# Wu0409/DuPL

Measured on AMD Instinct MI355X. Metric: training img/s at 448^2, VOC dual-student ViT-B/16, phase B step, higher is better.
Workload: dtype f32 storage / accumulation / results; Linear GEMMs (forward, dgrad, wgrad), attention (forward, backward) and the decoder convs as fp32-equivalent f16x3 split products on the f16 MFMA (operands as fp16 hi / lo planes, 3 products per block, fp32 accumulate; error vs fp64 <= the f32 MFMA kernels'); CA

## Files before the change

### dupl_amd/csrc/gemm_split.hip

```cpp
#include "common.h"
#include <type_traits>
#include "../../include/dupl_hip.h"

#ifndef G16_ABL
#define G16_ABL 0
#endif

namespace {

typedef _Float16 h8 __attribute__((ext_vector_type(8)));

constexpr int TBK = 32;
constexpr float LO_INV = 1.f / DUPL_LO_SCALE;

template <bool F1>
__global__ __launch_bounds__(256) void split_kernel(const float* __restrict__ x, __half* __restrict__ hi, __half* __restrict__ lo,
                                                    long n4, float scale) {
    for (long i = (long)blockIdx.x * blockDim.x + threadIdx.x; i < n4; i += (long)gridDim.x * blockDim.x) {
        const float4 v = reinterpret_cast<const float4*>(x)[i];
        __half h[4], l[4];
        if constexpr (F1) {
            split_f32_u(v.x * scale, h[0], l[0]);
            split_f32_u(v.y * scale, h[1], l[1]);
            split_f32_u(v.z * scale, h[2], l[2]);
// ... 44 lines not shown
#pragma unroll
            for (int e = 0; e < 16; ++e) {
                int row = rbase + (e & 3) + 8 * (e >> 2);
                asm volatile("" : "+v"(row));
                if (!interior && row >= p.M) continue;
                float v = (accM[i][j][e] + accX[i][j][e] * LO_INV) * alpha + bv;
                const bool w32 = p.c_rows <= 0 || row < p.c_rows;
                if (f_pre && w32) p.aux[(size_t)row * p.ldaux + col] = v;
                if (f_gelu) v = gelu_f(v);
                if (f_relu) v = fmaxf(v, 0.f);
                if (f_dgelu) v *= gelu_grad_f(p.aux[(size_t)row * p.ldaux + col]);
                if (f_rmask) v = p.aux[(size_t)row * p.ldaux + col] > 0.f ? v : 0.f;
                if (p.res) v += p.res[(size_t)row * p.ldr + col];
                if (f_acc) {
                    float* cp = p.C + (size_t)row * p.ldc + col;
                    if (ksplit > 1) unsafeAtomicAdd(cp, v);
                    else *cp += v;
                    continue;
                }
                amx = fmaxf(amx, fabsf(v));
                if (p.C && w32) p.C[(size_t)row * p.ldc + col] = v;
                if (Ch) {
                    __half h, l;
                    split_f32(v, h, l);
                    Ch[(size_t)row * p.ldo + col] = h;
                    Cl[(size_t)row * p.ldo + col] = l;
                }
            }
        }
    }
}


template <int WM, int WN, int WMP, bool SINGLE>
__device__ __forceinline__ void gemm16_epilogue_lds(const dupl_gemm16_desc& p, f32x16 (&accM)[WM][WN], f32x16 (&accX)[SINGLE ? 1 : WM][SINGLE ? 1 : WN],
                                                    float* __restrict__ tile, const int mw0, const int nw, const int lane,
                                                    const int ksplit, float& amx) {
    constexpr int TW = 32 * WN, TH = 32 * WMP, LPR = TW / 4, RPI = 64 / LPR;
    static_assert(WM % WMP == 0, "passes");
    const int l31 = lane & 31, hf = lane >> 5;
    const int fl = p.flags;
    const bool f_pre = fl & DUPL_GEMM_STORE_PRE, f_gelu = fl & DUPL_GEMM_GELU, f_relu = fl & DUPL_GEMM_RELU;
    const bool f_acc = fl & DUPL_GEMM_ACCUM, f_dgelu = fl & DUPL_GEMM_MUL_DGELU, f_rmask = fl & DUPL_GEMM_MUL_RELUMASK;
    const float alpha = (p.alpha_dev ? *p.alpha_dev : 1.f) * (p.post_scale != 0.f ? p.post_scale : 1.f);
    const float out_scale = p.out_exp > 0 ? ldexpf(1.f, p.out_exp) : 0.f;
#pragma unroll
    for (int ps = 0; ps < WM / WMP; ++ps) {
    const int mw = mw0 + ps * TH;
#pragma unroll
    for (int i = 0; i < WMP; ++i)
#pragma unroll
        for (int j = 0; j < WN; ++j)
#pragma unroll
            for (int e = 0; e < 16; ++e) {
                float v;
                if constexpr (SINGLE) v = accM[ps * WMP + i][j][e] * alpha;
                else v = (accM[ps * WMP + i][j][e] + accX[ps * WMP + i][j][e] * LO_INV) * alpha;
                tile[(i * 32 + (e & 3) + 8 * (e >> 2) + 4 * hf) * TW + j * 32 + l31] = v;
            }
    __half* Ch = static_cast<__half*>(p.C_hi);
    __half* Cl = static_cast<__half*>(p.C_lo);
    auto a16 = [](const void* q) { return (reinterpret_cast<uintptr_t>(q) & 15) == 0; };
    const bool vec = !(p.N & 3) && !(p.ldc & 3) && !(p.ldo & 3) && !(p.ldr & 3) && !(p.ldaux & 3) && a16(p.C) && a16(p.res) &&
                     a16(p.aux) && a16(p.bias) && !(reinterpret_cast<uintptr_t>(Ch) & 7) && !(reinterpret_cast<uintptr_t>(Cl) & 7);
    if (f_acc) {
        constexpr int RPA = 64 / TW;
        const int ca = lane % TW, ra = lane / TW;
        if (nw + ca >= p.N) continue;
        for (int r = ra; r < TH; r += RPA) {
            const int row = mw + r;
            if (row >= p.M) break;
            float* cp = p.C + (size_t)row * p.ldc + nw + ca;
            const float v = tile[r * TW + ca];
            if (ksplit > 1) unsafeAtomicAdd(cp, v);
            else *cp += v;
        }
        continue;
    }
    const int cl = (lane % LPR) * 4, rl = lane / LPR;
    const int col = nw + cl;
    const int nv = min(4, p.N - col);
    if (nv <= 0) continue;
    float bv[4] = {0.f, 0.f, 0.f, 0.f};
    if (p.bias) {
#pragma unroll
        for (int c = 0; c < 4; ++c)
            if (c < nv) bv[c] = p.bias[col + c];
    }
    const bool fast = vec && nv == 4;
    constexpr int EPU = 4;
    const bool need_aux = f_dgelu | f_rmask;
    for (int r0 = rl; r0 < TH; r0 += EPU * RPI) {
        f32x4 rq[EPU], aq[EPU];
        if (fast) {
#pragma unroll
            for (int u = 0; u < EPU; ++u) {
                const int r = r0 + u * RPI, row = mw + r;
                if (r < TH && row < p.M) {
                    if (p.res) rq[u] = *reinterpret_cast<const f32x4*>(p.res + (size_t)row * p.ldr + col);
                    if (need_aux) aq[u] = *reinterpret_cast<const f32x4*>(p.aux + (size_t)row * p.ldaux + col);
                }
            }
        }
#pragma unroll
        for (int u = 0; u < EPU; ++u) {
        const int r = r0 + u * RPI;
        if (r >= TH) break;
        const int row = mw + r;
        if (row >= p.M) break;
        const f32x4 t = *reinterpret_cast<const f32x4*>(tile + r * TW + cl);
        if (G16_ABL & 4) {
            if (t[0] + t[1] + t[2] + t[3] == 123.456f) p.C[0] = 1.f;
            continue;
        }
        float v[4] = {t[0] + bv[0], t[1] + bv[1], t[2] + bv[2], t[3] + bv[3]};
        float* auxp = p.aux + (size_t)row * p.ldaux + col;
        const bool w32 = p.c_rows <= 0 || row < p.c_rows;
        if (f_pre && w32) {
            if (fast) *reinterpret_cast<f32x4*>(auxp) = f32x4{v[0], v[1], v[2], v[3]};
            else
                {
_Pragma("unroll") for (int c = 0; c < 4; ++c) if (c < nv) auxp[c] = v[c]; }
        }
        if (f_gelu) gelu4(v);
        if (f_relu) {
#pragma unroll
            for (int c = 0; c < 4; ++c) v[c] = fmaxf(v[c], 0.f);
        }
        if (need_aux) {
            float a[4] = {0.f, 0.f, 0.f, 0.f};
            if (fast) {
                a[0] = aq[u][0]; a[1] = aq[u][1]; a[2] = aq[u][2]; a[3] = aq[u][3];
            } else
                {
_Pragma("unroll") for (int c = 0; c < 4; ++c) if (c < nv) a[c] = auxp[c]; }
            if (f_dgelu) gelu_grad_mul4(v, a);
            else {
#pragma unroll
                for (int c = 0; c < 4; ++c) v[c] = a[c] > 0.f ? v[c] : 0.f;
            }
        }
        if (p.res) {
            const float* rp = p.res + (size_t)row * p.ldr + col;
// ... 9 lines not shown
        if (p.C && w32) {
            float* cp = p.C + (size_t)row * p.ldc + col;
            if (fast) *reinterpret_cast<f32x4*>(cp) = f32x4{v[0], v[1], v[2], v[3]};
            else
                {
_Pragma("unroll") for (int c = 0; c < 4; ++c) if (c < nv) cp[c] = v[c]; }
        }
        if (Ch) {
            __half h[4], l[4];
            if (out_scale > 0.f) {
#pragma unroll
                for (int c = 0; c < 4; ++c) split_f32_u(v[c] * out_scale, h[c], l[c]);
            } else {
#pragma unroll
                for (int c = 0; c < 4; ++c) split_f32(v[c], h[c], l[c]);
            }
            __half* hp = Ch + (size_t)row * p.ldo + col;
            __half* lp = Cl + (size_t)row * p.ldo + col;
            if (fast) {
                *reinterpret_cast<uint2*>(hp) = *reinterpret_cast<const uint2*>(h);
                *reinterpret_cast<uint2*>(lp) = *reinterpret_cast<const uint2*>(l);
            } else
                {
_Pragma("unroll") for (int c = 0; c < 4; ++c)
                    if (c < nv) {
                        hp[c] = h[c];
                        lp[c] = l[c];
                    }
                }
        }
        }
    }
    }
}


struct Epi16 {
    bool f_pre, f_gelu, f_relu, f_dgelu, f_rmask, vec;
    float out_scale;
    __half *Ch, *Cl;
};
__device__ __forceinline__ Epi16 epi16_setup(const dupl_gemm16_desc& p) {
    Epi16 e;
    const int fl = p.flags;
    e.f_pre = fl & DUPL_GEMM_STORE_PRE; e.f_gelu = fl & DUPL_GEMM_GELU; e.f_relu = fl & DUPL_GEMM_RELU;
    e.f_dgelu = fl & DUPL_GEMM_MUL_DGELU; e.f_rmask = fl & DUPL_GEMM_MUL_RELUMASK;
    e.Ch = static_cast<__half*>(p.C_hi);
    e.Cl = static_cast<__half*>(p.C_lo);
    e.out_scale = p.out_exp > 0 ? ldexpf(1.f, p.out_exp) : 0.f;
    auto a16 = [](const void* q) { return (reinterpret_cast<uintptr_t>(q) & 15) == 0; };
    e.vec = !(p.N & 3) && !(p.ldc & 3) && !(p.ldo & 3) && !(p.ldr & 3) && !(p.ldaux & 3) && a16(p.C) && a16(p.res) && a16(p.aux) &&
            a16(p.bias) && !(reinterpret_cast<uintptr_t>(e.Ch) & 7) && !(reinterpret_cast<uintptr_t>(e.Cl) & 7);
    return e;
}
__device__ __forceinline__ void epi16_quad(const dupl_gemm16_desc& p, const Epi16& E, const int row, const int col, const int nv,
                                           const f32x4 t, const float (&bv)[4], float& amx, const f32x4 pre = f32x4{0.f, 0.f, 0.f, 0.f},
                                           const int pre_kind = 0) {
    const bool fast = E.vec && nv == 4;
    float v[4] = {t[0] + bv[0], t[1] + bv[1], t[2] + bv[2], t[3] + bv[3]};
    float* auxp = p.aux + (size_t)row * p.ldaux + col;
    const bool w32 = p.c_rows <= 0 || row < p.c_rows;
    if (E.f_pre && w32) {
        if (fast) *reinterpret_cast<f32x4*>(auxp) = f32x4{v[0], v[1], v[2], v[3]};
        else {
#pragma unroll
            for (int c = 0; c < 4; ++c) if (c < nv) auxp[c] = v[c];
// ... 217 lines not shown
            const int cs = s == 0 ? c0 : c1;
            h8 ah[WM], al[WM], bh[WN], bl[WN];
#pragma unroll
            for (int i = 0; i < WM; ++i) {
                ah[i] = *reinterpret_cast<const h8*>(st + a_row + i * 2048 + cs);
                al[i] = *reinterpret_cast<const h8*>(st + PA * 1024 + a_row + i * 2048 + cs);
            }
#pragma unroll
            for (int j = 0; j < WN; ++j) {
                bh[j] = *reinterpret_cast<const h8*>(st + b_row + j * 2048 + cs);
                bl[j] = *reinterpret_cast<const h8*>(st + PB * 1024 + b_row + j * 2048 + cs);
            }
#pragma unroll
            for (int i = 0; i < WM; ++i)
#pragma unroll
                for (int j = 0; j < WN; ++j) {
                    accM[i][j] = __builtin_amdgcn_mfma_f32_32x32x16_f16(ah[i], bh[j], accM[i][j], 0, 0, 0);
                    accX[i][j] = __builtin_amdgcn_mfma_f32_32x32x16_f16(ah[i], bl[j], accX[i][j], 0, 0, 0);
                    accX[i][j] = __builtin_amdgcn_mfma_f32_32x32x16_f16(al[i], bh[j], accX[i][j], 0, 0, 0);
                }
        }
    }

    float amx = 0.f;
    gemm16_epilogue<WM, WN>(p, accM, accX, m0 + wm * (32 * WM), n0 + wn * (32 * WN), m0 + BM <= p.M && n0 + BN <= p.N, l31, hf,
                            ksplit, amx);
    if (p.amax_out)
        gemm16_amax_flush(static_cast<unsigned int*>(p.amax_out), amx, reinterpret_cast<float*>(smem), threadIdx.x >> 6,
                          threadIdx.x & 63, NWM * NWN);
}


#define WAIT_LGKM0_VM(n) ((((n) & 15) | (((n) >> 4) << 14)) | (7 << 4))

template <int NMF, int NR, int R = 0>
__device__ __forceinline__ void sched_mfma_ds() {
    if constexpr (R < NR) {
        constexpr int nm = (R + 1) * NMF / NR - R * NMF / NR;
        if constexpr (nm > 0) __builtin_amdgcn_sched_group_barrier(0x008, nm, 0);
        __builtin_amdgcn_sched_group_barrier(0x100, 1, 0);
        sched_mfma_ds<NMF, NR, R + 1>();
    }
}
template <int NMF, int NR, int ND, int S = 0, int RD = 0, int DD = 0>
__device__ __forceinline__ void sched_mfma_ds_dma() {
    constexpr int NS = NR + ND;
    if constexpr (S < NS) {
        constexpr int nm = (S + 1) * NMF / NS - S * NMF / NS;
        if constexpr (nm > 0) __builtin_amdgcn_sched_group_barrier(0x008, nm, 0);
        constexpr bool rd = RD < NR && (DD >= ND || RD * ND <= DD * NR);
        if constexpr (rd) {
            __builtin_amdgcn_sched_group_barrier(0x100, 1, 0);
            sched_mfma_ds_dma<NMF, NR, ND, S + 1, RD + 1, DD>();
        } else {
            __builtin_amdgcn_sched_group_barrier(0x010, 1, 0);
            sched_mfma_ds_dma<NMF, NR, ND, S + 1, RD, DD + 1>();
        }
    }
}

template <int NR, int ND, int RD = 0, int DD = 0, class FR, class FD, class A, class B>
__device__ __forceinline__ void loads_b(FR& read_item, FD& dma_item, const char* st, const int cs, A& fa, B& fb, char* dst) {
    if constexpr (RD + DD < NR + ND) {
        constexpr bool rd = RD < NR && (DD >= ND || RD * ND <= DD * NR);
        if constexpr (rd) {
            read_item(std::integral_constant<int, RD>{}, st, cs, fa, fb);
// ... 187 lines not shown
        rb = nb;
    }

    asm volatile("s_waitcnt lgkmcnt(0)" ::: "memory");
    __builtin_amdgcn_s_barrier();
    asm volatile("" ::: "memory");
    constexpr int WMP = (NW * (32 * WM) * (32 * WN) * 4 <= STAGES * STAGE) ? WM : WM / 2;
    static_assert(NW * (32 * WMP) * (32 * WN) * 4 <= STAGES * STAGE, "epilogue tiles must fit the stages");
    if (G16_ABL & 16)
        if (tid == 0 && p.aux) reinterpret_cast<long long*>(p.aux)[(size_t)(blockIdx.x + gridDim.x * blockIdx.y) * 8 + 2] = clock64();
    if (G16_ABL & 8) {
        float sum = 0.f;
#pragma unroll
        for (int i = 0; i < WM; ++i)
#pragma unroll
            for (int j = 0; j < WN; ++j)
#pragma unroll
                for (int e = 0; e < 16; ++e) sum += accM[i][j][e] + (SINGLE ? 0.f : accX[SINGLE ? 0 : i][SINGLE ? 0 : j][e]);
        if (sum == 123.456f) p.C[0] = 1.f;
        return;
    }
    float amx = 0.f;
    gemm16_epilogue_lds<WM, WN, WMP, SINGLE>(p, accM, accX, reinterpret_cast<float*>(smem) + wave * ((32 * WMP) * (32 * WN)),
                                             m0 + wm * (32 * WM), n0 + wn * (32 * WN), lane, ksplit, amx);
    if (p.amax_out) gemm16_amax_flush(static_cast<unsigned int*>(p.amax_out), amx, reinterpret_cast<float*>(smem), wave, lane, NWM * NWN);
    if (G16_ABL & 16) {
        asm volatile("s_waitcnt vmcnt(0)" ::: "memory");
        if (tid == 0 && p.aux) {
            long long* q = reinterpret_cast<long long*>(p.aux) + (size_t)(blockIdx.x + gridDim.x * blockIdx.y) * 8;
            q[3] = clock64();
            q[5] = wall_clock64();
        }
    }
}


template <int WM, int WN, int NWM, int NWN, int WPS, bool SK = false, bool SINGLE = false, int STAGES = 3>
__global__ __launch_bounds__(64 * NWM * NWN, WPS) void gemm_f16x3_pring_kernel(const dupl_gemm16_desc p, const int g_gm) {
    constexpr int BM = 32 * WM * NWM, BN = 32 * WN * NWN, NW = NWM * NWN;
    constexpr int PA = BM / 16, PB = BN / 16;
    constexpr int NP = 2 * PA + 2 * PB;
    constexpr int STAGE = NP * 1024;
    constexpr int PPW = NP / NW;
    constexpr int NMF = 3 * WM * WN, NR = 2 * (WM + WN);
    constexpr int SIDE = NW * 2048;
    static_assert(NP % NW == 0, "pieces must divide over the waves");
    static_assert(STAGES * STAGE + SIDE <= 160 * 1024, "LDS");
    __shared__ __attribute__((aligned(1024))) char smem[STAGES * STAGE + SIDE];
    const int tid = threadIdx.x;
    const int lane = tid & 63, wave = __builtin_amdgcn_readfirstlane(tid >> 6);
    const int wm = wave / NWN, wn = wave % NWN;
    const int l31 = lane & 31, hf = lane >> 5;
    const int nbm = (p.M + BM - 1) / BM, nbn = (p.N + BN - 1) / BN;
    const int nblk = nbm * nbn;
    const int ntf = p.K / TBK;
    int nt = ntf;
    const int q8 = nblk >> 3, r8 = nblk & 7;
    const int gspan = g_gm * nbn;
    auto lid_origin = [&](const int lid, int& m0, int& n0) __attribute__((always_inline)) {
        const int gid = lid / gspan, gin = lid - gid * gspan;
        const int gfirst = gid * g_gm;
        const int gsz = min(nbm - gfirst, g_gm);
        m0 = (gfirst + gin % gsz) * BM;
        n0 = (gin / gsz) * BN;
    };
    auto tile_origin = [&](const int bid, int& m0, int& n0) __attribute__((always_inline)) {
// ... 164 lines not shown
        const int mw = m0 + wm * (32 * WM), nw = n0 + wn * (32 * WN);
        bool more;
        if constexpr (SK) {
            pos += nt;
            more = pos < pend;
            if (more) {
                nt = min(pend - pos, ntf);
                lid_origin(pos / ntf, m0, n0);
                plan(m0, n0, 0);
            }
        } else {
            bid += gridDim.x;
            more = has_tile(bid);
            if (more) {
                tile_origin(bid, m0, n0);
                plan(m0, n0, 0);
            }
        }
        if (more) {
#pragma unroll
            for (int s = 0; s < STAGES; ++s) issue(s);
        }
        gemm16_epilogue_side<WM, WN, SK, SINGLE>(p, accM, accX, reinterpret_cast<float*>(smem + STAGES * STAGE) + wave * 512, mw, nw, lane,
                                         amx);
        if (!more) break;
    }
    if (p.amax_out)
        gemm16_amax_flush(static_cast<unsigned int*>(p.amax_out), amx, reinterpret_cast<float*>(smem + STAGES * STAGE), wave, lane,
                          NWM * NWN);
}

typedef short s4v __attribute__((ext_vector_type(4)));
typedef _Float16 h4 __attribute__((ext_vector_type(4)));
template <int N, int I = 0, class F>
__device__ __forceinline__ void static_for(F&& f) {
    if constexpr (I < N) {
        f(std::integral_constant<int, I>{});
        static_for<N, I + 1>(f);
    }
}

constexpr bool slot_is_read(int S, int NR, int ND) {
    int rd = 0, dd = 0;
    for (int s = 0;; ++s) {
        const bool r = rd < NR && (dd >= ND || rd * ND <= dd * NR);
        if (s == S) return r;
        if (r) ++rd; else ++dd;
    }
}
constexpr int slot_index(int S, int NR, int ND) {
    int rd = 0, dd = 0;
    for (int s = 0;; ++s) {
        const bool r = rd < NR && (dd >= ND || rd * ND <= dd * NR);
        if (s == S) return r ? rd : dd;
        if (r) ++rd; else ++dd;
    }
}

template <int WM, int WN, int NWM, int NWN, int WPS, bool SK, int ACC, bool AKM, bool BKM, int STAGES = 3, bool ONESHOT = false>
__device__ __forceinline__ void gemm_f16x3_km_body(const dupl_gemm16_desc& p, const int g_gm, const int bid0, const int grid) {
    constexpr int BM = 32 * WM * NWM, BN = 32 * WN * NWN, NW = NWM * NWN;
    constexpr int PA = BM / 16, PB = BN / 16;
    constexpr int NP = 2 * PA + 2 * PB;
    constexpr int STAGE = NP * 1024;
    constexpr int PPW = NP / NW;
    constexpr int APW = 2 * PA / NW;
    constexpr int RBA = 2 * BM, RBB = 2 * BN;
    constexpr int NDA = AKM ? 2 : 1, NDB = BKM ? 2 : 1;
    constexpr int NIA = 2 * WM * NDA, NIB = 2 * WN * NDB;
    constexpr int NRI = NIA + NIB;
    constexpr int NMF = 3 * WM * WN;
    constexpr int SIDE = NW * 2048;
    static_assert(NP % NW == 0 && (2 * PA) % NW == 0, "pieces must divide over the waves, operand by operand");
    static_assert(STAGES * STAGE + SIDE <= 160 * 1024, "LDS");
// ... 346 lines not shown
                       ldexpf(1.f, scale_exp));
    return dupl_launch_status();
}

extern "C" int dupl_gemm_f16x3_group(const dupl_gemm16_desc* descs, int32_t n, dupl_stream_t stream) {
    if (!descs || n < 1 || n > DUPL_GEMM16_GROUP_MAX) return DUPL_ERR_ARG;
    g16_group_args g;
    g.n = n;
    int total = 0, group = 0;
    auto al16 = [](const void* q) { return (reinterpret_cast<uintptr_t>(q) & 15) == 0; };
    for (int i = 0; i < n; ++i) {
        const dupl_gemm16_desc& d = descs[i];
        if (d.struct_size != sizeof(dupl_gemm16_desc)) return DUPL_ERR_ARG;
        if (!d.A_hi || !d.A_lo || !d.B_hi || !d.B_lo || !d.C || d.C_hi || d.C_lo || d.bias || d.res || d.c_rows || d.amax_out ||
            d.M <= 0 || d.N <= 0 || d.K <= 0)
            return DUPL_ERR_ARG;
        if (d.flags != DUPL_GEMM_ACCUM || d.fmt != 1 || d.a_layout != 1 || d.b_layout != 1 || (d.K % TBK) || d.K / TBK < 3 ||
            (d.lda % 8) || (d.ldb % 8) || (d.M & 7) || (d.N & 7) || d.ka_valid < 0 || d.kb_valid < 0 || d.ka_valid > d.K ||
            d.kb_valid > d.K || d.group < 0 || d.group > 4096)
            return DUPL_ERR_ARG;
        if (!al16(d.A_hi) || !al16(d.A_lo) || !al16(d.B_hi) || !al16(d.B_lo)) return DUPL_ERR_ARG;
        g.d[i] = d;
        g.first[i] = total;
        const int nblk = ((d.M + 255) / 256) * ((d.N + 127) / 128);
        total += nblk;
        if (d.group) group = d.group;
    }
    g.first[n] = total;
    DUPL_LAUNCH((gemm_f16x3_km_group_kernel<2, 2, 4, 2, 2>), dim3((unsigned)(8 * ((total + 7) / 8))), dim3(512), 0, (hipStream_t)stream, g,
                       group ? group : G16_GROUP_RING);
    return dupl_launch_status();
}

extern "C" int dupl_gemm_f16x3(const dupl_gemm16_desc* d, dupl_stream_t stream) {
    if (!d || d->struct_size != sizeof(dupl_gemm16_desc)) return DUPL_ERR_ARG;
    if (!d->A_hi || !d->A_lo || !d->B_hi || !d->B_lo || d->M <= 0 || d->N <= 0 || d->K <= 0) return DUPL_ERR_ARG;
    if ((d->K % TBK) || (d->lda % 8) || (d->ldb % 8)) return DUPL_ERR_ARG;
    if (d->tile < 0 || d->concurrency < 0 || d->concurrency > 8 || d->group < 0 || d->group > 4096 || d->persist_blocks < 0 ||
        d->persist_blocks > 1024 || (d->persist_blocks & 7))
        return DUPL_ERR_ARG;
    {
        const int t = d->tile;
        if (t != 0 && t != 3 && t != 5 && t != 6 && t != 7 && t != 8 && t != 10 && t != 11 && t != 12 && t != 14) return DUPL_ERR_ARG;
    }
    const int g16_tile = d->tile, g16_concurrency = d->concurrency > 0 ? d->concurrency : 1;
    const int g16_persist_blocks = d->persist_blocks ? d->persist_blocks : (g16_concurrency >= 2 ? 192 : 256);
    const int g16_group_m = d->group ? d->group : G16_GROUP_M, g16_group_ring = d->group ? d->group : G16_GROUP_RING;
    const int g16_f1_big_from = G16_F1_BIG_FROM;
    auto al16 = [](const void* q) { return (reinterpret_cast<uintptr_t>(q) & 15) == 0; };
    if (!al16(d->A_hi) || !al16(d->A_lo) || !al16(d->B_hi) || !al16(d->B_lo)) return DUPL_ERR_ARG;
    if (!d->C && !d->C_hi) return DUPL_ERR_ARG;
    if ((d->C_hi == nullptr) != (d->C_lo == nullptr)) return DUPL_ERR_ARG;
    if ((d->flags & (DUPL_GEMM_STORE_PRE | DUPL_GEMM_MUL_DGELU | DUPL_GEMM_MUL_RELUMASK)) && !d->aux) return DUPL_ERR_ARG;
    if (d->flags & ~(DUPL_GEMM_GELU | DUPL_GEMM_RELU | DUPL_GEMM_STORE_PRE | DUPL_GEMM_ACCUM | DUPL_GEMM_MUL_DGELU |
                     DUPL_GEMM_MUL_RELUMASK))
        return DUPL_ERR_ARG;
    const bool accum = d->flags & DUPL_GEMM_ACCUM;
    if (accum && (!d->C || d->C_hi || d->bias || d->res || d->c_rows)) return DUPL_ERR_ARG;
    if (d->c_rows < 0 || (d->c_rows && (d->flags & (DUPL_GEMM_MUL_DGELU | DUPL_GEMM_MUL_RELUMASK)))) return DUPL_ERR_ARG;
    if (d->amax_out && (accum || d->c_rows || (reinterpret_cast<uintptr_t>(d->amax_out) & 3))) return DUPL_ERR_ARG;
    const bool kmajor = d->a_layout || d->b_layout;
    if (d->fmt < 0 || d->fmt > 1 || d->out_exp < 0 || d->out_exp > 15 || (d->out_exp && d->fmt != 1) ||
        (d->fmt == 1 && !kmajor && (accum || d->amax_out)))
        return DUPL_ERR_ARG;
    hipStream_t s = (hipStream_t)stream;
    int ksplit = 1;
    if (accum) {
        const long tiles = (long)((d->M + 127) / 128) * ((d->N + 127) / 128);
        ksplit = (int)((512 + tiles - 1) / tiles);
        const int maxs = (d->K / TBK + 7) / 8;
        if (ksplit > maxs) ksplit = maxs;
        if (ksplit < 1) ksplit = 1;
        if (d->deterministic) ksplit = 1;
    }
    int tile = g16_tile;
    if (tile == 0) {
// ... 19 lines not shown
        if ((d->a_layout ? d->ka_valid : 0) > d->K || (d->b_layout ? d->kb_valid : 0) > d->K) return DUPL_ERR_ARG;
        if (!d->a_layout && d->ka_valid) return DUPL_ERR_ARG;
        if (!d->b_layout && d->kb_valid) return DUPL_ERR_ARG;
        const int nb21 = ((d->M + 255) / 256) * ((d->N + 127) / 128);
        const bool sk = accum && !d->deterministic && ksplit > 1;
        dupl_gemm16_desc dsk = *d;
        if (accum) {
            const int ntf = d->K / TBK;
            auto per = [&](int s_) { return (ntf + s_ - 1) / s_; };
            auto fits = [&](int s_) { return s_ > 0 && (long)nb21 * s_ <= g16_persist_blocks && per(s_) >= 3 && ntf - (s_ - 1) * per(s_) >= 3; };
            if (dsk.sk_slices > 0 && !fits(dsk.sk_slices)) dsk.sk_slices = 0;
            if (dsk.sk_slices == 0) {
                int S = nb21 > g16_persist_blocks ? -1 : g16_persist_blocks / nb21;
                while (S > 1 && (per(S) < 3 || ntf - (S - 1) * per(S) < 3)) --S;
                dsk.sk_slices = S;
            }
            if (dsk.sk_slices > 0 && !fits(dsk.sk_slices)) dsk.sk_slices = -1;
        }
        if (accum && !d->a_layout) {
            if (!d->b_layout || d->deterministic) return DUPL_ERR_ARG;
            DUPL_LAUNCH((gemm_f16x3_km_kernel<2, 2, 4, 2, 2, true, 1, false, true>), dim3((unsigned)g16_persist_blocks), dim3(512), 0, s, dsk, g16_group_ring);
        } else if (accum) {
            if (!(d->a_layout && d->b_layout)) return DUPL_ERR_ARG;
            if (sk) DUPL_LAUNCH((gemm_f16x3_km_kernel<2, 2, 4, 2, 2, true, 1, true, true>), dim3((unsigned)g16_persist_blocks), dim3(512), 0, s, dsk, g16_group_ring);
            else DUPL_LAUNCH((gemm_f16x3_km_kernel<2, 2, 4, 2, 2, false, 2, true, true>), persist_grid(nb21), dim3(512), 0, s, *d, g16_group_ring);
        } else {
            if (d->a_layout || !d->b_layout) return DUPL_ERR_ARG;
            DUPL_LAUNCH((gemm_f16x3_km_kernel<2, 2, 4, 2, 2, false, 0, false, true>), persist_grid(nb21), dim3(512), 0, s, *d, g16_group_ring);
        }
        return dupl_launch_status();
    }
    if (d->fmt == 1) {
        const int nb22 = ((d->M + 255) / 256) * ((d->N + 255) / 256), nb21 = ((d->M + 255) / 256) * ((d->N + 127) / 128);
        int t = (g16_tile == 8 || g16_tile == 12 || g16_tile == 14) ? g16_tile : (nb22 >= g16_f1_big_from ? 8 : 12);
        if (d->K / TBK < 3 && t == 14) t = 12;
        if (t == 8) {
            const int cn = (d->N + 255) / 256, rm = (d->M + 255) / 256, cus = 256;
            const int full = nb22 / cus, tail = nb22 - full * cus;
            const int r_big = full > 0 ? (full * cus) / cn : 0;
            if (g16_tile == 0 && full > 0 && tail > 0 && tail * 10 < cus * 3 && r_big > 0 && r_big < rm && !d->amax_out) {
                const int M1 = r_big * 256;
                dupl_gemm16_desc d1 = *d, d2 = *d;
                d1.M = M1;
                d2.M = d->M - M1;
                auto adv = [&](const void* q, size_t elems, size_t bytes) { return q ? static_cast<const void*>(static_cast<const char*>(q) + elems * bytes) : nullptr; };
                d2.A_hi = adv(d->A_hi, (size_t)M1 * d->lda, 2); d2.A_lo = adv(d->A_lo, (size_t)M1 * d->lda, 2);
                d2.C = (float*)adv(d->C, (size_t)M1 * d->ldc, 4);
                d2.C_hi = (void*)adv(d->C_hi, (size_t)M1 * d->ldo, 2); d2.C_lo = (void*)adv(d->C_lo, (size_t)M1 * d->ldo, 2);
                d2.res = (const float*)adv(d->res, (size_t)M1 * d->ldr, 4);
                d2.aux = (float*)adv(d->aux, (size_t)M1 * d->ldaux, 4);
                if (d->c_rows > 0) {
                    if (d->c_rows <= M1) {
                        d2.c_rows = 0; d2.C = nullptr; d2.aux = nullptr; d2.flags &= ~DUPL_GEMM_STORE_PRE;
                    } else { d1.c_rows = 0; d2.c_rows = d->c_rows - M1; }
                }
                if (d2.C || d2.C_hi) {
                    DUPL_LAUNCH((gemm_f16x3_ring_kernel<4, 2, 2, 4, 2, 2, true>), dim3((unsigned)(r_big * cn)), dim3(512), 0, s, d1, g16_group_ring);
                    DUPL_LAUNCH((gemm_f16x3_ring_kernel<2, 2, 4, 2, 2, 3, true>),
                                       dim3((unsigned)(((d2.M + 255) / 256) * ((d2.N + 127) / 128))), dim3(512), 0, s, d2, g16_group_ring);
                    return dupl_launch_status();
                }
            }
            DUPL_LAUNCH((gemm_f16x3_ring_kernel<4, 2, 2, 4, 2, 2, true>), blocks(256, 256), dim3(512), 0, s, *d, g16_group_ring);
        }
        else if (t == 12) DUPL_LAUNCH((gemm_f16x3_ring_kernel<2, 2, 4, 2, 2, 3, true>), blocks(256, 128), dim3(512), 0, s, *d, g16_group_ring);
        else
            DUPL_LAUNCH((gemm_f16x3_pring_kernel<2, 2, 4, 2, 2, false, true, 3>), persist_grid(nb21), dim3(512), 0, s, *d, g16_group_ring);
        return dupl_launch_status();
    }
    if (tile == 10 && (accum || d->K / TBK < 3)) tile = 6;
    if (tile == 11 && (!accum || d->deterministic || d->K / TBK < 8)) tile = accum ? 5 : 6;
    if (tile == 11) {
        DUPL_LAUNCH((gemm_f16x3_pring_kernel<2, 2, 4, 2, 2, true>), dim3((unsigned)g16_persist_blocks), dim3(512), 0, s, *d,
                           g16_group_ring);
        return dupl_launch_status();
    }
    if (tile == 10) {
        const int nblk = ((d->M + 255) / 256) * ((d->N + 127) / 128);
        const int tx = (nblk + 7) / 8, bmax = g16_persist_blocks / 8;
        const int rounds = (tx + bmax - 1) / bmax;
        const int grid = 8 * ((tx + rounds - 1) / rounds);
        DUPL_LAUNCH((gemm_f16x3_pring_kernel<2, 2, 4, 2, 2>), dim3((unsigned)grid), dim3(512), 0, s, *d, g16_group_ring);
        return dupl_launch_status();
    }
    if (tile == 8 || tile == 9 || tile == 12 || tile == 14) tile = 5;
    if (tile == 6) DUPL_LAUNCH((gemm_f16x3_ring_kernel<2, 2, 4, 2, 2>), blocks(256, 128), dim3(512), 0, s, *d, g16_group_ring);
    else if (tile == 7) DUPL_LAUNCH((gemm_f16x3_ring_kernel<4, 2, 2, 2, 1>), blocks(256, 128), dim3(256), 0, s, *d, g16_group_ring);
    else if (tile == 3) DUPL_LAUNCH((gemm_f16x3_kernel<2, 1, 2, 2, 2>), blocks(128, 64), dim3(256), 0, s, *d, g16_group_m);
    else DUPL_LAUNCH((gemm_f16x3_kernel<2, 1, 2, 4, 4>), blocks(128, 128), dim3(512), 0, s, *d, g16_group_m);
    return dupl_launch_status();
}
```

Baseline: 77.83.

## Add 16x16x32 MFMA ring GEMM kernel for fmt1 split-f16 path and make it default

Adds a new ring-buffered f16x3 GEMM kernel that uses 16x16x32 f16 MFMA instructions. It has its own LDS layout, a phase-interleaved fragment schedule with sched_group_barrier hints, and a rotated LDS epilogue to reduce bank conflicts. It becomes the default for the fmt==1 GEMMs, including the row-split big/tail launch, and the old kernels stay reachable via tiles 8 and 12. The shared epilogue is refactored into a row writer with a pluggable park step. The intent is higher MFMA throughput and better LDS/compute overlap, at the risk of register pressure or a worse schedule than the tuned 32x32 kernel.

New measurement: 80.54, median of 6. 1.03x the previous value.

```diff
diff --git a/dupl_amd/csrc/gemm_split.hip b/dupl_amd/csrc/gemm_split.hip
--- a/dupl_amd/csrc/gemm_split.hip
+++ b/dupl_amd/csrc/gemm_split.hip
@@ -100,32 +100,19 @@
 }
 
 
-template <int WM, int WN, int WMP, bool SINGLE>
-__device__ __forceinline__ void gemm16_epilogue_lds(const dupl_gemm16_desc& p, f32x16 (&accM)[WM][WN], f32x16 (&accX)[SINGLE ? 1 : WM][SINGLE ? 1 : WN],
-                                                    float* __restrict__ tile, const int mw0, const int nw, const int lane,
-                                                    const int ksplit, float& amx) {
-    constexpr int TW = 32 * WN, TH = 32 * WMP, LPR = TW / 4, RPI = 64 / LPR;
-    static_assert(WM % WMP == 0, "passes");
-    const int l31 = lane & 31, hf = lane >> 5;
+template <int TW, int TH, int NPS, bool ROT, class Park>
+__device__ __forceinline__ void gemm16_epilogue_rows(const dupl_gemm16_desc& p, Park&& park, float* __restrict__ tile, const int mw0,
+                                                     const int nw, const int lane, const int ksplit, float& amx) {
+    constexpr int LPR = TW / 4, RPI = 64 / LPR;
+    auto at = [](const int r, const int c) { return r * TW + (ROT ? ((c + ((r >> 2) & 1) * 16) & (TW - 1)) : c); };
     const int fl = p.flags;
     const bool f_pre = fl & DUPL_GEMM_STORE_PRE, f_gelu = fl & DUPL_GEMM_GELU, f_relu = fl & DUPL_GEMM_RELU;
     const bool f_acc = fl & DUPL_GEMM_ACCUM, f_dgelu = fl & DUPL_GEMM_MUL_DGELU, f_rmask = fl & DUPL_GEMM_MUL_RELUMASK;
-    const float alpha = (p.alpha_dev ? *p.alpha_dev : 1.f) * (p.post_scale != 0.f ? p.post_scale : 1.f);
     const float out_scale = p.out_exp > 0 ? ldexpf(1.f, p.out_exp) : 0.f;
 #pragma unroll
-    for (int ps = 0; ps < WM / WMP; ++ps) {
+    for (int ps = 0; ps < NPS; ++ps) {
     const int mw = mw0 + ps * TH;
-#pragma unroll
-    for (int i = 0; i < WMP; ++i)
-#pragma unroll
-        for (int j = 0; j < WN; ++j)
-#pragma unroll
-            for (int e = 0; e < 16; ++e) {
-                float v;
-                if constexpr (SINGLE) v = accM[ps * WMP + i][j][e] * alpha;
-                else v = (accM[ps * WMP + i][j][e] + accX[ps * WMP + i][j][e] * LO_INV) * alpha;
-                tile[(i * 32 + (e & 3) + 8 * (e >> 2) + 4 * hf) * TW + j * 32 + l31] = v;
-            }
+    park(ps);
     __half* Ch = static_cast<__half*>(p.C_hi);
     __half* Cl = static_cast<__half*>(p.C_lo);
     auto a16 = [](const void* q) { return (reinterpret_cast<uintptr_t>(q) & 15) == 0; };
@@ -139,7 +126,7 @@
             const int row = mw + r;
             if (row >= p.M) break;
             float* cp = p.C + (size_t)row * p.ldc + nw + ca;
-            const float v = tile[r * TW + ca];
+            const float v = tile[at(r, ca)];
             if (ksplit > 1) unsafeAtomicAdd(cp, v);
             else *cp += v;
         }
@@ -176,7 +163,7 @@
         if (r >= TH) break;
         const int row = mw + r;
         if (row >= p.M) break;
-        const f32x4 t = *reinterpret_cast<const f32x4*>(tile + r * TW + cl);
+        const f32x4 t = *reinterpret_cast<const f32x4*>(tile + at(r, cl));
         if (G16_ABL & 4) {
             if (t[0] + t[1] + t[2] + t[3] == 123.456f) p.C[0] = 1.f;
             continue;
@@ -252,6 +239,49 @@
         }
     }
     }
+}
+
+template <int WM, int WN, int WMP, bool SINGLE>
+__device__ __forceinline__ void gemm16_epilogue_lds(const dupl_gemm16_desc& p, f32x16 (&accM)[WM][WN], f32x16 (&accX)[SINGLE ? 1 : WM][SINGLE ? 1 : WN],
+                                                    float* __restrict__ tile, const int mw0, const int nw, const int lane,
+                                                    const int ksplit, float& amx) {
+    constexpr int TW = 32 * WN, TH = 32 * WMP;
+    static_assert(WM % WMP == 0, "passes");
+    const int l31 = lane & 31, hf = lane >> 5;
+    const float alpha = (p.alpha_dev ? *p.alpha_dev : 1.f) * (p.post_scale != 0.f ? p.post_scale : 1.f);
+    auto park = [&](const int ps) __attribute__((always_inline)) {
+#pragma unroll
+        for (int i = 0; i < WMP; ++i)
+#pragma unroll
+            for (int j = 0; j < WN; ++j)
+#pragma unroll
+                for (int e = 0; e < 16; ++e) {
+                    float v;
+                    if constexpr (SINGLE) v = accM[ps * WMP + i][j][e] * alpha;
+                    else v = (accM[ps * WMP + i][j][e] + accX[ps * WMP + i][j][e] * LO_INV) * alpha;
+                    tile[(i * 32 + (e & 3) + 8 * (e >> 2) + 4 * hf) * TW + j * 32 + l31] = v;
+                }
+    };
+    gemm16_epilogue_rows<TW, TH, WM / WMP, false>(p, park, tile, mw0, nw, lane, ksplit, amx);
+}
+
+template <int RB, int CB, int RBP>
+__device__ __forceinline__ void gemm16_epilogue_lds16(const dupl_gemm16_desc& p, f32x4 (&acc)[RB][CB], float* __restrict__ tile,
+                                                      const int mw0, const int nw, const int lane, const int ksplit, float& amx) {
+    constexpr int TW = 16 * CB, TH = 16 * RBP;
+    static_assert(RB % RBP == 0 && TW == 64, "passes; the rotation is laid out for 64-float rows");
+    const int l15 = lane & 15, q = lane >> 4;
+    const float alpha = (p.alpha_dev ? *p.alpha_dev : 1.f) * (p.post_scale != 0.f ? p.post_scale : 1.f);
+    auto park = [&](const int ps) __attribute__((always_inline)) {
+#pragma unroll
+        for (int i = 0; i < RBP; ++i)
+#pragma unroll
+            for (int j = 0; j < CB; ++j)
+#pragma unroll
+                for (int e = 0; e < 4; ++e)
+                    tile[(i * 16 + 4 * q + e) * TW + ((j * 16 + l15 + (q & 1) * 16) & (TW - 1))] = acc[ps * RBP + i][j][e] * alpha;
+    };
+    gemm16_epilogue_rows<TW, TH, RB / RBP, true>(p, park, tile, mw0, nw, lane, ksplit, amx);
 }
 
 
@@ -535,6 +565,14 @@
 
 
 #define WAIT_LGKM0_VM(n) ((((n) & 15) | (((n) >> 4) << 14)) | (7 << 4))
+
+template <int N, int I = 0, class F>
+__device__ __forceinline__ void static_for(F&& f) {
+    if constexpr (I < N) {
+        f(std::integral_constant<int, I>{});
+        static_for<N, I + 1>(f);
+    }
+}
 
 template <int NMF, int NR, int R = 0>
 __device__ __forceinline__ void sched_mfma_ds() {
@@ -788,6 +826,180 @@
             q[5] = wall_clock64();
         }
     }
+}
+
+
+template <int WM, int WN, int NWM, int NWN, int WPS, int STAGES>
+__global__ __launch_bounds__(64 * NWM * NWN, WPS) void gemm_f16x3_ring16_kernel(const dupl_gemm16_desc p, const int g_gm) {
+    constexpr int BM = 32 * WM * NWM, BN = 32 * WN * NWN, NW = NWM * NWN;
+    constexpr int PA = BM / 16, PB = BN / 16;
+    constexpr int NP = 2 * PA + 2 * PB;
+    constexpr int STAGE = NP * 1024;
+    constexpr int PPW = NP / NW;
+    constexpr int RB = 2 * WM, CB = 2 * WN;
+    constexpr int NPH = WM;
+    constexpr int NMF = 3 * 2 * CB;
+    static_assert(NP % NW == 0, "pieces must divide over the waves");
+    static_assert(STAGES * STAGE <= 160 * 1024, "LDS");
+    static_assert((STAGES - 1) * PPW <= 63, "vmcnt range");
+    static_assert(NPH % 2 == 0, "the A fragment sets alternate by phase");
+    __shared__ __attribute__((aligned(1024))) char smem[STAGES * STAGE];
+    const int tid = threadIdx.x;
+    const int lane = tid & 63, wave = __builtin_amdgcn_readfirstlane(tid >> 6);
+    const int wm = wave / NWN, wn = wave % NWN;
+
+    const int nbm = (p.M + BM - 1) / BM, nbn = (p.N + BN - 1) / BN;
+    const int nblk = nbm * nbn;
+    const int bid = blockIdx.x;
+    const int q8 = nblk >> 3, r8 = nblk & 7;
+    const int xcd = bid & 7, idx = bid >> 3;
+    const int lid = (xcd < r8 ? xcd * (q8 + 1) : r8 * (q8 + 1) + (xcd - r8) * q8) + idx;
+    const int gspan = g_gm * nbn;
+    const int gid = lid / gspan, gin = lid - gid * gspan;
+    const int gfirst = gid * g_gm;
+    const int gsz = min(nbm - gfirst, g_gm);
+    const int tm = gfirst + gin % gsz, tn = gin / gsz;
+    const int m0 = tm * BM, n0 = tn * BN;
+    const int nt = p.K / TBK;
+
+    const int prow = lane >> 2;
+    const int jsrc = (lane & 3) ^ ((4 - (prow >> 2)) & 3);
+    const char* gp[PPW];
+#pragma unroll
+    for (int i = 0; i < PPW; ++i) {
+        const int g = wave + NW * i;
+        const __half* plane;
+        int ld, r0, R, q;
+        if (g < PA) { plane = static_cast<const __half*>(p.A_hi); ld = p.lda; r0 = m0; R = p.M; q = g; }
+        else if (g < 2 * PA) { plane = static_cast<const __half*>(p.A_lo); ld = p.lda; r0 = m0; R = p.M; q = g - PA; }
+        else if (g < 2 * PA + PB) { plane = static_cast<const __half*>(p.B_hi); ld = p.ldb; r0 = n0; R = p.N; q = g - 2 * PA; }
+        else { plane = static_cast<const __half*>(p.B_lo); ld = p.ldb; r0 = n0; R = p.N; q = g - 2 * PA - PB; }
+        const int row = min(r0 + q * 16 + prow, R - 1);
+        gp[i] = reinterpret_cast<const char*>(plane + (size_t)row * ld) + jsrc * 16;
+    }
+    auto dma_item = [&](auto dc, char* dst) __attribute__((always_inline)) {
+        constexpr int I = decltype(dc)::value;
+        __builtin_amdgcn_global_load_lds((const __attribute__((address_space(1))) void*)gp[I],
+                                         (__attribute__((address_space(3))) void*)(dst + I * (NW * 1024)), 16, 0, 0);
+        gp[I] += TBK * 2;
+    };
+    auto issue = [&](int buf) __attribute__((always_inline)) {
+        static_for<PPW>([&](auto i) __attribute__((always_inline)) { dma_item(i, smem + buf * STAGE + wave * 1024); });
+    };
+
+    const int l15 = lane & 15;
+    const int ch = ((lane >> 4) ^ ((4 - (l15 >> 2)) & 3)) * 16;
+    const int a_off = (wm * (32 * WM) + l15) * 64 + ch, b_off = 2 * PA * 1024 + (wn * (32 * WN) + l15) * 64 + ch;
+
+    f32x4 acc[RB][CB];
+#pragma unroll
+    for (int i = 0; i < RB; ++i)
+#pragma unroll
+        for (int j = 0; j < CB; ++j) acc[i][j] = f32x4{0.f, 0.f, 0.f, 0.f};
+    h8 fa0[4], fa1[4], fb[2 * CB];
+    auto read_a = [&](auto rc, const char* st, const int ph, h8(&fa)[4]) __attribute__((always_inline)) {
+        constexpr int R = decltype(rc)::value;
+        fa[R] = *reinterpret_cast<const h8*>(st + (R >> 1) * (PA * 1024) + a_off + (2 * ph + (R & 1)) * 1024);
+    };
+    auto read_b = [&](auto jc, const char* st) __attribute__((always_inline)) {
+        constexpr int J = decltype(jc)::value;
+        fb[J] = *reinterpret_cast<const h8*>(st + b_off + J * 1024);
+        fb[CB + J] = *reinterpret_cast<const h8*>(st + PB * 1024 + b_off + J * 1024);
+    };
+    auto mfma6 = [&](auto phc, auto jc, const h8(&fa)[4]) __attribute__((always_inline)) {
+        constexpr int PH = decltype(phc)::value, J = decltype(jc)::value;
+#pragma unroll
+        for (int k = 0; k < 2; ++k) acc[2 * PH + k][J] = __builtin_amdgcn_mfma_f32_16x16x32_f16(fa[k], fb[J], acc[2 * PH + k][J], 0, 0, 0);
+#pragma unroll
+        for (int k = 0; k < 2; ++k) acc[2 * PH + k][J] = __builtin_amdgcn_mfma_f32_16x16x32_f16(fa[k], fb[CB + J], acc[2 * PH + k][J], 0, 0, 0);
+#pragma unroll
+        for (int k = 0; k < 2; ++k) acc[2 * PH + k][J] = __builtin_amdgcn_mfma_f32_16x16x32_f16(fa[2 + k], fb[J], acc[2 * PH + k][J], 0, 0, 0);
+    };
+    constexpr int S_MFMA = 0x008, S_DSR = 0x100, S_VMEM = 0x010;
+    auto hint6 = [](auto nrd) __attribute__((always_inline)) {
+        constexpr int NRD = decltype(nrd)::value;
+        static_for<NRD>([](auto) __attribute__((always_inline)) {
+            __builtin_amdgcn_sched_group_barrier(S_MFMA, 1, 0);
+            __builtin_amdgcn_sched_group_barrier(S_DSR, 1, 0);
+        });
+        __builtin_amdgcn_sched_group_barrier(S_MFMA, 6 - NRD, 0);
+    };
+    auto inner_phases = [&](const char* st) __attribute__((always_inline)) {
+        static_for<NPH - 1>([&](auto ph) __attribute__((always_inline)) {
+            constexpr int PH = decltype(ph)::value;
+            static_for<CB>([&](auto j) __attribute__((always_inline)) {
+                constexpr int J = decltype(j)::value;
+                constexpr int NRD = (J < 2 ? 2 : 0) + (PH == 0 && J == 0 ? 2 : 0);
+                if constexpr (PH == 0 && J == 0) read_b(std::integral_constant<int, CB - 1>{}, st);
+                if constexpr (J < 2) {
+                    read_a(std::integral_constant<int, 2 * J>{}, st, PH + 1, PH & 1 ? fa0 : fa1);
+                    read_a(std::integral_constant<int, 2 * J + 1>{}, st, PH + 1, PH & 1 ? fa0 : fa1);
+                }
+                mfma6(ph, j, PH & 1 ? fa1 : fa0);
+                hint6(std::integral_constant<int, NRD>{});
+            });
+        });
+    };
+    auto last_phase = [&](auto loadc, auto dmac, const char* nx, char* dst) __attribute__((always_inline)) {
+        constexpr bool LOAD = decltype(loadc)::value, DMA = decltype(dmac)::value;
+        constexpr auto ph = std::integral_constant<int, NPH - 1>{};
+        static_for<CB>([&](auto j) __attribute__((always_inline)) {
+            constexpr int J = decltype(j)::value;
+            constexpr int D0 = J * PPW / CB, D1 = (J + 1) * PPW / CB;
+            if constexpr (LOAD) {
+                if constexpr (J == 0) static_for<4>([&](auto r) __attribute__((always_inline)) { read_a(r, nx, 0, fa0); });
+                else read_b(std::integral_constant<int, J - 1>{}, nx);
+            }
+            if constexpr (DMA) static_for<D1 - D0>([&](auto i) __attribute__((always_inline)) {
+                dma_item(std::integral_constant<int, D0 + decltype(i)::value>{}, dst);
+            });
+            mfma6(ph, j, fa1);
+            hint6(std::integral_constant<int, LOAD ? (J == 0 ? 4 : 2) : 0>{});
+            if constexpr (DMA && D1 > D0) __builtin_amdgcn_sched_group_barrier(S_VMEM, D1 - D0, 0);
+        });
+    };
+#pragma unroll
+    for (int s = 0; s < STAGES; ++s)
+        if (s < nt) issue(s);
+    if (nt >= STAGES) asm volatile("s_waitcnt vmcnt(%0)" ::"n"((STAGES - 1) * PPW) : "memory");
+    else asm volatile("s_waitcnt vmcnt(0)" ::: "memory");
+    __builtin_amdgcn_s_barrier();
+    asm volatile("" ::: "memory");
+    static_for<4>([&](auto r) __attribute__((always_inline)) { read_a(r, smem, 0, fa0); });
+    static_for<CB - 1>([&](auto j) __attribute__((always_inline)) { read_b(j, smem); });
+    int rb = 0;
+    int t = 0;
+    for (; t + STAGES < nt; ++t) {
+        const int nb = rb + 1 == STAGES ? 0 : rb + 1;
+        inner_phases(smem + rb * STAGE);
+        __builtin_amdgcn_sched_barrier(0);
+        __builtin_amdgcn_s_waitcnt(WAIT_LGKM0_VM((STAGES - 2) * PPW));
+        __builtin_amdgcn_s_barrier();
+        asm volatile("" ::: "memory");
+        last_phase(std::true_type{}, std::true_type{}, smem + nb * STAGE, smem + rb * STAGE + wave * 1024);
+        rb = nb;
+    }
+    for (; t + 1 < nt; ++t) {
+        const int nb = rb + 1 == STAGES ? 0 : rb + 1;
+        inner_phases(smem + rb * STAGE);
+        __builtin_amdgcn_sched_barrier(0);
+        __builtin_amdgcn_s_waitcnt(WAIT_LGKM0_VM(0));
+        __builtin_amdgcn_s_barrier();
+        asm volatile("" ::: "memory");
+        last_phase(std::true_type{}, std::false_type{}, smem + nb * STAGE, nullptr);
+        rb = nb;
+    }
+    inner_phases(smem + rb * STAGE);
+    last_phase(std::false_type{}, std::false_type{}, nullptr, nullptr);
+
+    asm volatile("s_waitcnt lgkmcnt(0)" ::: "memory");
+    __builtin_amdgcn_s_barrier();
+    asm volatile("" ::: "memory");
+    constexpr int RBP = (NW * (16 * RB) * (16 * CB) * 4 <= STAGES * STAGE) ? RB : RB / 2;
+    static_assert(NW * (16 * RBP) * (16 * CB) * 4 <= STAGES * STAGE, "epilogue tiles must fit the stages");
+    float amx = 0.f;
+    gemm16_epilogue_lds16<RB, CB, RBP>(p, acc, reinterpret_cast<float*>(smem) + wave * ((16 * RBP) * (16 * CB)), m0 + wm * (32 * WM),
+                                       n0 + wn * (32 * WN), lane, 1, amx);
 }
 
 
@@ -1018,14 +1230,6 @@
 
 typedef short s4v __attribute__((ext_vector_type(4)));
 typedef _Float16 h4 __attribute__((ext_vector_type(4)));
-template <int N, int I = 0, class F>
-__device__ __forceinline__ void static_for(F&& f) {
-    if constexpr (I < N) {
-        f(std::integral_constant<int, I>{});
-        static_for<N, I + 1>(f);
-    }
-}
-
 constexpr bool slot_is_read(int S, int NR, int ND) {
     int rd = 0, dd = 0;
     for (int s = 0;; ++s) {
@@ -1438,6 +1642,24 @@
     return dupl_launch_status();
 }
 
+static bool g16_split_rows(const dupl_gemm16_desc& d, const int M1, dupl_gemm16_desc& d1, dupl_gemm16_desc& d2) {
+    d1 = d; d2 = d;
+    d1.M = M1;
+    d2.M = d.M - M1;
+    auto adv = [&](const void* q, size_t elems, size_t bytes) { return q ? static_cast<const void*>(static_cast<const char*>(q) + elems * bytes) : nullptr; };
+    d2.A_hi = adv(d.A_hi, (size_t)M1 * d.lda, 2); d2.A_lo = adv(d.A_lo, (size_t)M1 * d.lda, 2);
+    d2.C = (float*)adv(d.C, (size_t)M1 * d.ldc, 4);
+    d2.C_hi = (void*)adv(d.C_hi, (size_t)M1 * d.ldo, 2); d2.C_lo = (void*)adv(d.C_lo, (size_t)M1 * d.ldo, 2);
+    d2.res = (const float*)adv(d.res, (size_t)M1 * d.ldr, 4);
+    d2.aux = (float*)adv(d.aux, (size_t)M1 * d.ldaux, 4);
+    if (d.c_rows > 0) {
+        if (d.c_rows <= M1) {
+            d2.c_rows = 0; d2.C = nullptr; d2.aux = nullptr; d2.flags &= ~DUPL_GEMM_STORE_PRE;
+        } else { d1.c_rows = 0; d2.c_rows = d.c_rows - M1; }
+    }
+    return d2.C || d2.C_hi;
+}
+
 extern "C" int dupl_gemm_f16x3(const dupl_gemm16_desc* d, dupl_stream_t stream) {
     if (!d || d->struct_size != sizeof(dupl_gemm16_desc)) return DUPL_ERR_ARG;
     if (!d->A_hi || !d->A_lo || !d->B_hi || !d->B_lo || d->M <= 0 || d->N <= 0 || d->K <= 0) return DUPL_ERR_ARG;
@@ -1447,7 +1669,7 @@
         return DUPL_ERR_ARG;
     {
         const int t = d->tile;
-        if (t != 0 && t != 3 && t != 5 && t != 6 && t != 7 && t != 8 && t != 10 && t != 11 && t != 12 && t != 14) return DUPL_ERR_ARG;
+        if (t != 0 && t != 3 && t != 5 && t != 6 && t != 7 && t != 8 && t != 10 && t != 11 && t != 12 && t != 14 && t != 18 && t != 22) return DUPL_ERR_ARG;
     }
     const int g16_tile = d->tile, g16_concurrency = d->concurrency > 0 ? d->concurrency : 1;
     const int g16_persist_blocks = d->persist_blocks ? d->persist_blocks : (g16_concurrency >= 2 ? 192 : 256);
@@ -1533,37 +1755,23 @@
     }
     if (d->fmt == 1) {
         const int nb22 = ((d->M + 255) / 256) * ((d->N + 255) / 256), nb21 = ((d->M + 255) / 256) * ((d->N + 127) / 128);
-        int t = (g16_tile == 8 || g16_tile == 12 || g16_tile == 14) ? g16_tile : (nb22 >= g16_f1_big_from ? 8 : 12);
+        int t = (g16_tile == 8 || g16_tile == 12 || g16_tile == 14 || g16_tile == 18 || g16_tile == 22) ? g16_tile
+                                                                                                         : (nb22 >= g16_f1_big_from ? 18 : 22);
         if (d->K / TBK < 3 && t == 14) t = 12;
-        if (t == 8) {
+        if (t == 18) {
             const int cn = (d->N + 255) / 256, rm = (d->M + 255) / 256, cus = 256;
             const int full = nb22 / cus, tail = nb22 - full * cus;
             const int r_big = full > 0 ? (full * cus) / cn : 0;
-            if (g16_tile == 0 && full > 0 && tail > 0 && tail * 10 < cus * 3 && r_big > 0 && r_big < rm && !d->amax_out) {
-                const int M1 = r_big * 256;
-                dupl_gemm16_desc d1 = *d, d2 = *d;
-                d1.M = M1;
-                d2.M = d->M - M1;
-                auto adv = [&](const void* q, size_t elems, size_t bytes) { return q ? static_cast<const void*>(static_cast<const char*>(q) + elems * bytes) : nullptr; };
-                d2.A_hi = adv(d->A_hi, (size_t)M1 * d->lda, 2); d2.A_lo = adv(d->A_lo, (size_t)M1 * d->lda, 2);
-                d2.C = (float*)adv(d->C, (size_t)M1 * d->ldc, 4);
-                d2.C_hi = (void*)adv(d->C_hi, (size_t)M1 * d->ldo, 2); d2.C_lo = (void*)adv(d->C_lo, (size_t)M1 * d->ldo, 2);
-                d2.res = (const float*)adv(d->res, (size_t)M1 * d->ldr, 4);
-                d2.aux = (float*)adv(d->aux, (size_t)M1 * d->ldaux, 4);
-                if (d->c_rows > 0) {
-                    if (d->c_rows <= M1) {
-                        d2.c_rows = 0; d2.C = nullptr; d2.aux = nullptr; d2.flags &= ~DUPL_GEMM_STORE_PRE;
-                    } else { d1.c_rows = 0; d2.c_rows = d->c_rows - M1; }
-                }
-                if (d2.C || d2.C_hi) {
-                    DUPL_LAUNCH((gemm_f16x3_ring_kernel<4, 2, 2, 4, 2, 2, true>), dim3((unsigned)(r_big * cn)), dim3(512), 0, s, d1, g16_group_ring);
-                    DUPL_LAUNCH((gemm_f16x3_ring_kernel<2, 2, 4, 2, 2, 3, true>),
-                                       dim3((unsigned)(((d2.M + 255) / 256) * ((d2.N + 127) / 128))), dim3(512), 0, s, d2, g16_group_ring);
-                    return dupl_launch_status();
-                }
-            }
-            DUPL_LAUNCH((gemm_f16x3_ring_kernel<4, 2, 2, 4, 2, 2, true>), blocks(256, 256), dim3(512), 0, s, *d, g16_group_ring);
-        }
+            dupl_gemm16_desc d1, d2;
+            if (g16_tile == 0 && full > 0 && tail > 0 && tail * 10 < cus * 3 && r_big > 0 && r_big < rm && !d->amax_out &&
+                g16_split_rows(*d, r_big * 256, d1, d2)) {
+                DUPL_LAUNCH((gemm_f16x3_ring16_kernel<4, 2, 2, 4, 2, 2>), dim3((unsigned)(r_big * cn)), dim3(512), 0, s, d1, g16_group_ring);
+                DUPL_LAUNCH((gemm_f16x3_ring16_kernel<2, 2, 4, 2, 2, 3>), dim3((unsigned)(((d2.M + 255) / 256) * ((d2.N + 127) / 128))),
+                            dim3(512), 0, s, d2, g16_group_ring);
+            } else DUPL_LAUNCH((gemm_f16x3_ring16_kernel<4, 2, 2, 4, 2, 2>), blocks(256, 256), dim3(512), 0, s, *d, g16_group_ring);
+        }
+        else if (t == 22) DUPL_LAUNCH((gemm_f16x3_ring16_kernel<2, 2, 4, 2, 2, 3>), blocks(256, 128), dim3(512), 0, s, *d, g16_group_ring);
+        else if (t == 8) DUPL_LAUNCH((gemm_f16x3_ring_kernel<4, 2, 2, 4, 2, 2, true>), blocks(256, 256), dim3(512), 0, s, *d, g16_group_ring);
         else if (t == 12) DUPL_LAUNCH((gemm_f16x3_ring_kernel<2, 2, 4, 2, 2, 3, true>), blocks(256, 128), dim3(512), 0, s, *d, g16_group_ring);
         else
             DUPL_LAUNCH((gemm_f16x3_pring_kernel<2, 2, 4, 2, 2, false, true, 3>), persist_grid(nb21), dim3(512), 0, s, *d, g16_group_ring);
@@ -1584,7 +1792,7 @@
         DUPL_LAUNCH((gemm_f16x3_pring_kernel<2, 2, 4, 2, 2>), dim3((unsigned)grid), dim3(512), 0, s, *d, g16_group_ring);
         return dupl_launch_status();
     }
-    if (tile == 8 || tile == 9 || tile == 12 || tile == 14) tile = 5;
+    if (tile == 8 || tile == 9 || tile == 12 || tile == 14 || tile == 18 || tile == 22) tile = 5;
     if (tile == 6) DUPL_LAUNCH((gemm_f16x3_ring_kernel<2, 2, 4, 2, 2>), blocks(256, 128), dim3(512), 0, s, *d, g16_group_ring);
     else if (tile == 7) DUPL_LAUNCH((gemm_f16x3_ring_kernel<4, 2, 2, 2, 1>), blocks(256, 128), dim3(256), 0, s, *d, g16_group_ring);
     else if (tile == 3) DUPL_LAUNCH((gemm_f16x3_kernel<2, 1, 2, 2, 2>), blocks(128, 64), dim3(256), 0, s, *d, g16_group_m);
```
